# p3achyjr/p3achygo

Measured on AMD Instinct MI355X. Metric: self-play positions/sec at 1/8 MI355X, b12c256btl3 19x19 n=32, higher is better.
Workload: dtype f16; 1 GPU; b12c256btl3 random-init, self-play: C++ host (Gumbel MCTS n=32, default k<=5, selected k=5) -> p3hip_run over batches of 1024 leaf positions -> results back to the search; one step = one round = one engine batch of each of the 8 game groups = 8192 positions; batch_per_gpu=1024, concurrent_games_per_gpu=8192, game_groups_per_gpu=8, lanes_per_group=1, ladder_node_budget=0, parallelism=games sharded x1, no collective

## Files before the change

p3achygo_amd/csrc/engine.cpp:

```cpp
#include <hip/hip_runtime.h>
#include <chrono>

#include <atomic>
#include <cmath>
#include <cstdio>
#include <cstdlib>
#include <cstring>
#include <functional>
#include <map>
#include <memory>
#include <unordered_set>
#include <string>
#include <vector>

#include "../../include/p3hip.h"
#include "kernels.h"
#include "lconv_i8.h"
#include "slot_state.h"
#include "symmetry.h"
#include "transformer.h"

namespace {

constexpr float kBnEps = 1e-3f;
constexpr int kNLoc = 361;
constexpr size_t kFeatBytes = sizeof(p3hip_features);
static_assert(sizeof(p3hip_features) == 1860, "p3hip_features layout");
static_assert(sizeof(p3hip_result) == 4 * 1892, "p3hip_result layout");

thread_local std::string g_create_error;

struct Tensor {
  std::vector<int> dims;
  const float* data;
  size_t size() const {
    size_t n = 1;
    for (int d : dims) n *= d;
    return n;
  }
};

struct WeightFile {
  int version = 0, nblocks = 0, C = 0, Cb = 0, H = 0, V = 0, bint = 0, inner = 0, btype = 0;
  int model_C = 0;
  std::vector<std::vector<float>> padded;
  std::vector<float> data;
  std::map<std::string, Tensor> tensors;

  bool load(const char* path, std::string& err) {
    FILE* f = fopen(path, "rb");
    if (!f) { err = std::string("cannot open ") + path; return false; }
    char magic[4];
    int hdr[10];
    if (fread(magic, 1, 4, f) != 4 || memcmp(magic, "P3W1", 4) != 0 || fread(hdr, 4, 10, f) != 10) {
      err = "not a .p3w file"; fclose(f); return false;
    }
    version = hdr[0]; nblocks = hdr[1]; C = hdr[2]; Cb = hdr[3]; H = hdr[4]; V = hdr[5];
    bint = hdr[6]; inner = hdr[7]; btype = hdr[8];
    int nt = hdr[9];
    if (nt < 1 || nt > 8192 || nblocks < 1 || nblocks > 256 || (btype == 3 ? bint != 0 : bint < 1)) {
      err = "implausible .p3w header"; fclose(f); return false;
    }
    struct Ent { char name[48]; int ndim; int dims[4]; long long off; };
    std::vector<Ent> ents(nt);
    long long total = 0;
    for (auto& e : ents) {
      if (fread(e.name, 1, 48, f) != 48 || fread(&e.ndim, 4, 1, f) != 1 ||
          fread(e.dims, 4, 4, f) != 4 || fread(&e.off, 8, 1, f) != 1) {
        err = "truncated tensor table"; fclose(f); return false;
      }
      long long sz = 1;
      bool ok = e.ndim >= 0 && e.ndim <= 4 && e.off >= 0 && e.off < (1ll << 31);
      for (int d = 0; ok && d < e.ndim; ++d) {
        ok = e.dims[d] > 0 && e.dims[d] < (1 << 24);
        sz *= e.dims[d];
        ok = ok && sz < (1ll << 31);
      }
      if (!ok) { err = "corrupt tensor table"; fclose(f); return false; }
      if (e.off + sz > total) total = e.off + sz;
    }
    long pos = ftell(f);
    pos += (64 - pos % 64) % 64;
    fseek(f, pos, SEEK_SET);
    data.resize(total);
    if (fread(data.data(), 4, total, f) != (size_t)total) { err = "truncated data"; fclose(f); return false; }
    fclose(f);
    for (auto& e : ents) {
      Tensor t;
      t.dims.assign(e.dims, e.dims + e.ndim);
      t.data = data.data() + e.off;
      tensors[std::string(e.name, strnlen(e.name, sizeof e.name))] = t;
    }
    model_C = C;
    if (btype == 3 && p3::tfm_supported(C, Cb) && p3::tfm_stream_width(C) != C) pad_transformer_io(p3::tfm_stream_width(C));
    return true;
  }
  void pad_transformer_io(int Cp) {
    auto pad = [&](const std::string& n, size_t rows, bool out_channels) {
      auto it = tensors.find(n);
      const size_t want = out_channels ? rows * C : (size_t)C * 32;
      if (it == tensors.end() || it->second.size() != want) return;
      std::vector<float> w(out_channels ? rows * Cp : (size_t)Cp * 32, 0.0f);
      for (size_t i = 0; i < want; ++i) {
        const size_t r = out_channels ? i / C : 0, c = out_channels ? i % C : i;
        w[out_channels ? r * Cp + c : c] = it->second.data[i];
      }
      padded.push_back(std::move(w));
      Tensor t;
      t.dims = it->second.dims;
      t.dims.back() = out_channels ? Cp : t.dims.back();
      if (!out_channels) t.dims[t.dims.size() - 2] = Cp;
      t.data = padded.back().data();
      it->second = t;
    };
    pad("init_conv.w", 25 * 15, true);
    pad("init_game.w", 8, true);
    pad("init_game.b", 1, true);
    for (const char* n : {"policy.conv_p.w", "policy.conv_g.w", "value.conv.w"}) pad(n, 0, false);
    C = Cp;
  }
  mutable std::string missing;
  mutable std::vector<std::vector<float>> zeros;
  mutable std::map<std::string, Tensor> stand_ins;
  const Tensor& get(const std::string& n, size_t expect = 0) const {
    auto it = tensors.find(n);
    if (it != tensors.end() && (expect == 0 || it->second.size() == expect)) return it->second;
    if (missing.size() < 400) missing += (missing.empty() ? "" : ", ") + n + (it == tensors.end() ? "" : " (wrong size)");
    auto st = stand_ins.find(n);
    if (st != stand_ins.end()) return st->second;
    zeros.emplace_back(expect ? expect : 1, 0.0f);
    Tensor t;
    t.dims = {(int)zeros.back().size()};
    t.data = zeros.back().data();
    return stand_ins[n] = t;
  }
  bool is_broadcast(int i) const { return bint > 0 && i % bint == bint - 1; }
};

struct Arena {
  std::vector<unsigned char> host;
  bool bad_stream = false;
  size_t add(const void* p, size_t bytes) {
    size_t off = (host.size() + 255) & ~size_t(255);
    host.resize(off + bytes);
    memcpy(host.data() + off, p, bytes);
    return off;
  }
};

void pack_segment(std::vector<_Float16>& dst, const float* W, int taps, int ntaps_pad,
                  int cin_total, int cout_total, int cin0, int CB, int cout0, int CP) {
  for (int tap = 0; tap < ntaps_pad; ++tap)
    for (int q = 0; q < CB / 16; ++q)
      for (int h = 0; h < 2; ++h)
        for (int co = 0; co < CP; ++co)
          for (int e = 0; e < 8; ++e) {
            int ci = cin0 + q * 16 + h * 8 + e, c = cout0 + co;
            float v = 0.0f;
            if (tap < taps && ci < cin_total && c < cout_total)
              v = W[((size_t)tap * cin_total + ci) * cout_total + c];
            dst.push_back((_Float16)v);
          }
}

void pack_segment_3x3(std::vector<_Float16>& dst, const float* W, int cin_total, int cout_total, int CB, int CP) {
  for (int ky = 0; ky < 3; ++ky)
    for (int q32 = 0; q32 < CB / 32; ++q32)
      for (int kx = 0; kx < 3; ++kx)
        for (int q = 2 * q32; q < 2 * q32 + 2; ++q)
          for (int h = 0; h < 2; ++h)
            for (int co = 0; co < CP; ++co)
              for (int e = 0; e < 8; ++e) {
                const int ci = q * 16 + h * 8 + e, tap = ky * 3 + kx;
                float v = 0.0f;
                if (ci < cin_total && co < cout_total) v = W[((size_t)tap * cin_total + ci) * cout_total + co];
                dst.push_back((_Float16)v);
              }
}

void pack_granule(std::vector<_Float16>& dst, const float* W, int cin_total, int cout_total, int tap, int k0, int cout0,
                  const float* scale) {
  for (int j = 0; j < 2; ++j)
    for (int c = 0; c < 2; ++c)
      for (int h = 0; h < 2; ++h)
        for (int n = 0; n < 32; ++n)
          for (int el = 0; el < 8; ++el) {
            const int co = cout0 + 32 * c + n;
            float v = W[((size_t)tap * cin_total + k0 + 16 * j + 8 * h + el) * cout_total + co];
            if (scale) v *= scale[co];
            dst.push_back((_Float16)v);
          }
}

struct FoldedBN { size_t scale_off, shift_off; };

void pack_afrag(std::vector<_Float16>& dst, const float* W, int K, int N, int ld, int col0) {
  for (int ct = 0; ct < N / 16; ++ct)
    for (int st = 0; st < K / 32; ++st)
      for (int lane = 0; lane < 64; ++lane)
        for (int el = 0; el < 8; ++el)
          dst.push_back((_Float16)W[(size_t)(32 * st + 8 * (lane >> 4) + el) * ld + col0 + 16 * ct + (lane & 15)]);
}

void spiral_rope_table(int D, double* cos_out, double* sin_out) {
  const int K = 4, per = D / K, nth = D / 4;
  const double kPi = 3.14159265358979323846;
  std::vector<double> theta(D);
  for (int i = 0; i < D; ++i) {
    const int k = i / per, r = (i % per) / 2;
    int t = 2 * (k % (K / 2)) + (r / 2) * K + (r % 2);
    if (t > nth - 1) t = nth - 1;
    theta[i] = std::pow(100.0, -(double)t / nth);
  }
  for (int s = 0; s < kNLoc; ++s)
    for (int i = 0; i < D; ++i) {
      const double ang = (i / per) * (kPi / K);
      const double proj = (s / 19) * std::cos(ang) + (s % 19) * std::sin(ang);
      cos_out[s * D + i] = std::cos(theta[i] * proj);
      sin_out[s * D + i] = std::sin(theta[i] * proj);
    }
}

struct LayerPlan {
  int kw, cin, cout;
  bool pre, act, res, dual;
  FoldedBN pre_bn, out_bn;
  int in_buf, out_buf, out2_buf;
  size_t stream_off = 0;
  int nms = 0;
  size_t q_off = 0, qs_off = 0;
  int qidx = -1;
};

struct TfmPlan { size_t rms_in = 0, rms_out = 0, wqkv = 0, wo = 0, wgu = 0, wdown = 0; };

struct BlockPlan {
  int kind;
  TfmPlan tfm;
  std::vector<LayerPlan> layers;
  size_t stream_off = 0;
  int nms = 0;
  size_t stream_bytes = 0;
  FoldedBN bn[p3::kMaxBlockLayers];
  size_t stream2_off = 0, stream3_off = 0;
  int nms2 = 0, nms3 = 0;
  size_t dense_bias_off = 0;
  bool first_fused = false, last_fused = false;
  bool dense_fused = false;
  int head_of = -1, tail_of = -1;
  size_t head_bytes = 0, tail_bytes = 0;
};

struct Pass {
  const unsigned char* feats = nullptr;
  int npos = 0;
  float* out = nullptr;
  float* res = nullptr;
  int* timed = nullptr;
};

}

struct p3hip_engine {
  std::string path, err;
  int batch = 0, device = 0;
  uint32_t flags = 0;
  WeightFile wf;
  int n_cu = 256;
  bool c128_wg8 = false;
  bool runs_contiguous = false;
  bool bcast_fuse = true;
  int stop_block = -1;
  bool fuse = true, join = true;
  int stagger = -1;
  bool pair_turns = true;
  bool direct_results = true;
  bool time_run = false;
  bool blockw = false;
  bool blockw_diag = false;
  struct BlockwRun { size_t first; int nblk; size_t stream_off, prm_off; };
  std::vector<BlockwRun> bw_runs;
  hipModule_t bw_mod = nullptr;
  hipFunction_t bw_fn = nullptr;
  unsigned long long* d_bw_stamps = nullptr;
  hipStream_t stream = nullptr;
  hipGraph_t graph = nullptr;
  hipGraphExec_t graph_exec = nullptr;
  bool graph_failed = false, graph_warm = false;
  Pass graph_pass;
  std::vector<hipEvent_t> blk_ev;

  unsigned char* d_arena = nullptr;
  std::vector<BlockPlan> blocks;
  size_t init_stream_off = 0; int init_nms = 0;
  size_t game_w_off = 0, game_b_off = 0;
  size_t heads_stream_off = 0; int heads_nms = 0;
  size_t heads_conv_a_off = 0, heads_image_off = 0;
  bool tfm = false;
  int tfm_heads = 0, tfm_D = 0;
  size_t rope_cos_off = 0, rope_sin_off = 0;
  bool int8 = false, calibrating = false, have_scales = false;
  int n_q = 0;
  unsigned* d_amax = nullptr;
  float* d_ascale = nullptr;
  std::vector<float> h_scale;
  bool sym = false;
  uint32_t sym_mask = 0xFF;
  int sym_k = 8;
  int sym_syms[p3::kNumSyms] = {0, 1, 2, 3, 4, 5, 6, 7};
  int rows = 0;
  unsigned char* d_sfeats = nullptr;
  float* d_cout = nullptr;
  bool heads_fused = false;
  std::map<std::string, size_t> head_off;

  unsigned char* h_feats = nullptr;
  unsigned char* h_feats_compact = nullptr;
  unsigned char* d_feats = nullptr;
  _Float16 *d_x = nullptr, *d_t = nullptr, *d_u = nullptr;
  _Float16* d_qkv = nullptr;
#ifdef P3_DIAG
  unsigned long long* d_stamps = nullptr;
  unsigned long long* d_spans = nullptr;
  int launch_index = 0;
#endif
  _Float16* d_s = nullptr;
  float* d_hp = nullptr;
  float* d_out = nullptr;
  float* h_out = nullptr;
  float* d_res = nullptr;
  double t_h2d = 0, t_fwd = 0, t_d2h = 0;
  long t_runs = 0;
  bool feats_identity = false;
  p3::SlotStates slots;
  int last_n = 0;
  std::vector<unsigned char> slot_sym, row_sym;

  struct DeviceCache {
    bool on = false;
    unsigned mask = 0, run = 0;
    unsigned long long* d_tkeys = nullptr;
    unsigned* d_tmeta = nullptr;
    float* d_tvals = nullptr;
    p3::CacheKey* h_slot_keys = nullptr;
    p3::CacheKey *h_keys = nullptr, *d_keys = nullptr;
    int *h_hit = nullptr, *d_hit = nullptr, *h_victim = nullptr, *d_victim = nullptr;
    int *h_lists = nullptr, *d_lists = nullptr;
    unsigned *h_sym = nullptr, *d_sym = nullptr;
    unsigned char* d_feats2 = nullptr;
    std::vector<int> out_row;
    std::vector<unsigned char> was_hit;
    unsigned long long lookups = 0, hits = 0, inserts = 0;
  } cache;
  int out_row_of(int slot) const {
    const int row = slots.row(slot);
    return (row >= 0 && cache.on) ? cache.out_row[row] : row;
  }

  bool check(hipError_t e, const char* what) {
    if (e == hipSuccess) return true;
    err = std::string(what) + ": " + hipGetErrorString(e);
    return false;
  }
  template <class T>
  const T* dev(size_t off) const { return reinterpret_cast<const T*>(d_arena + off); }
  bool bind() { return check(hipSetDevice(device), "hipSetDevice"); }
};

namespace {

FoldedBN fold_bn(Arena& ar, const WeightFile& wf, const std::string& prefix, size_t n) {
  const Tensor& g = wf.get(prefix + ".gamma", n);
  const Tensor& b = wf.get(prefix + ".beta", n);
  const Tensor& m = wf.get(prefix + ".mean", n);
  const Tensor& v = wf.get(prefix + ".var", n);
  std::vector<float> sc(n), sh(n);
  for (size_t i = 0; i < n; ++i) {
    sc[i] = g.data[i] / std::sqrt(v.data[i] + kBnEps);
    sh[i] = b.data[i] - m.data[i] * sc[i];
  }
  FoldedBN f;
  f.scale_off = ar.add(sc.data(), n * 4);
  f.shift_off = ar.add(sh.data(), n * 4);
  return f;
}

size_t add_stream(Arena& ar, const std::vector<_Float16>& s, int& nms, int cout_pass) {
  const size_t ms = (size_t)cout_pass * 128;
  if (s.size() * 2 % ms != 0) ar.bad_stream = true;
  nms = (int)(s.size() * 2 / ms);
  return ar.add(s.data(), s.size() * 2);
}

bool build_plan(p3hip_engine* e, Arena& ar) {
  const WeightFile& wf = e->wf;
  const int C = wf.C, Cb = wf.Cb;
  const bool fused = (C == 256 && Cb == 128) || (C == 128 && Cb == 64);
  const bool classic = wf.btype == 2 && C == 192 && wf.inner == 2;
  const bool bottleneck_ok = wf.btype == 1 || (wf.btype == 0 && wf.inner >= 1 && wf.inner <= 3);
  const bool layerwise = (C == 384 && Cb == 192 && bottleneck_ok) || classic;
  const bool v_ok = wf.V == 32 || wf.V == 48 || wf.V == 64 || wf.V == 80;
  const bool tfm = wf.btype == 3 && p3::tfm_supported(wf.model_C, Cb) && C == p3::tfm_stream_width(wf.model_C) &&
                   (C == 384 || p3::heads_fusable(C, wf.V));
  if ((!((fused && bottleneck_ok) || layerwise) && !tfm) || wf.H != 32 || !v_ok) {
    e->err = "unsupported architecture for the HIP engine (need (C, Cb) in {(128,64), (256,128), (384,192)} with "
             "btl (1-3 inner layers) or nbt blocks, or C=192 classic blocks of two convs, or a transformer trunk "
             "(" P3HIP_TRANSFORMER_SET "); H=32, V in {32,48,64,80} (transformer: V in {32,48,64}, and 80 at d > 256))";
    return false;
  }
  e->tfm = tfm;
  if (tfm) {
    e->tfm_heads = Cb;
    e->tfm_D = wf.model_C / Cb;
  }
  if (e->int8 && !layerwise) {
    e->err = "INT8 is available only for layer-wise trunks (C = 384 / C_b = 192 btl or nbt blocks, C = 192 classic "
             "blocks); this trunk runs fused block kernels or the transformer";
    return false;
  }
  const int CB = classic ? 64 : ((layerwise || tfm) ? 128 : Cb);
  const int CPI = classic ? 64 : 128;
  {
    std::vector<_Float16> s;
    const Tensor& w = wf.get("init_conv.w", (size_t)25 * 15 * C);
    for (int cp = 0; cp < C / CPI; ++cp)
      pack_segment(s, w.data, 25, 28, 15, C, 0, 16, cp * CPI, CPI);
    e->init_stream_off = add_stream(ar, s, e->init_nms, CPI);
    e->game_w_off = ar.add(wf.get("init_game.w", (size_t)8 * C).data, 8 * C * 4);
    e->game_b_off = ar.add(wf.get("init_game.b", (size_t)C).data, C * 4);
  }
  {
    static const bool want_blockw = getenv("P3HIP_BLOCKW") != nullptr && atoi(getenv("P3HIP_BLOCKW")) != 0;
    e->blockw = want_blockw && C == 256 && Cb == 128 && wf.btype == 0 && wf.inner >= 1 && wf.inner <= 3;
    if (e->blockw) e->bcast_fuse = false;
  }
  bool have_xa = false;
  std::vector<std::pair<size_t, std::vector<_Float16>>> run_streams;
  std::vector<_Float16> head_stream, tail_stream;
  int head_of = -1, tail_of = -1;
  std::vector<std::function<void()>> layout;
  auto flush_run = [&]() {
    if (!run_streams.empty()) {
      auto rs_all = std::make_shared<std::vector<std::pair<size_t, std::vector<_Float16>>>>(std::move(run_streams));
      auto hs = std::make_shared<std::vector<_Float16>>(std::move(head_stream));
      auto ts = std::make_shared<std::vector<_Float16>>(std::move(tail_stream));
      const int h_of = head_of, t_of = tail_of;
      layout.push_back([&ar, e, rs_all, hs, ts, h_of, t_of, Cb]() {
        int nms_unused = 0;
        if (h_of >= 0) {
          add_stream(ar, *hs, nms_unused, Cb);
          BlockPlan& b = e->blocks[rs_all->front().first];
          b.head_of = h_of;
          b.head_bytes = hs->size() * 2;
          e->blocks[h_of].last_fused = true;
        }
        for (auto& rs : *rs_all) {
          BlockPlan& b = e->blocks[rs.first];
          b.stream_off = add_stream(ar, rs.second, b.nms, Cb);
          b.stream_bytes = rs.second.size() * 2;
        }
        if (t_of >= 0) {
          add_stream(ar, *ts, nms_unused, Cb);
          BlockPlan& b = e->blocks[rs_all->back().first];
          b.tail_of = t_of;
          b.tail_bytes = ts->size() * 2;
        }
      });
    }
    run_streams.clear();
    head_stream.clear();
    tail_stream.clear();
    head_of = tail_of = -1;
  };
  if (tfm) {
    std::vector<double> cd(kNLoc * e->tfm_D), sd(kNLoc * e->tfm_D);
    spiral_rope_table(e->tfm_D, cd.data(), sd.data());
    const std::vector<float> cf(cd.begin(), cd.end()), sf(sd.begin(), sd.end());
    e->rope_cos_off = ar.add(cf.data(), cf.size() * 4);
    e->rope_sin_off = ar.add(sf.data(), sf.size() * 4);
  }
  for (int i = 0; tfm && i < wf.nblocks; ++i) {
    const std::string p = "blocks." + std::to_string(i);
    const int c = wf.model_C, f = 2 * c;
    auto T = [&](const char* n, size_t sz) { return wf.get(p + "." + n, sz).data; };
    BlockPlan bp;
    bp.kind = 5;
    bp.tfm.rms_in = ar.add(T("rms_in.scale", c), c * 4);
    bp.tfm.rms_out = ar.add(T("rms_out.scale", c), c * 4);
    std::vector<_Float16> w;
    for (const char* n : {"q.w", "k.w", "v.w"}) pack_afrag(w, T(n, (size_t)c * c), c, c, c, 0);
    bp.tfm.wqkv = ar.add(w.data(), w.size() * 2);
    w.clear();
    pack_afrag(w, T("o.w", (size_t)c * c), c, c, c, 0);
    bp.tfm.wo = ar.add(w.data(), w.size() * 2);
    w.clear();
    pack_afrag(w, T("ffn_gate.w", (size_t)c * f), c, f, f, 0);
    pack_afrag(w, T("ffn_up.w", (size_t)c * f), c, f, f, 0);
    bp.tfm.wgu = ar.add(w.data(), w.size() * 2);
    w.clear();
    pack_afrag(w, T("ffn_down.w", (size_t)f * c), f, c, c, 0);
    bp.tfm.wdown = ar.add(w.data(), w.size() * 2);
    e->blocks.push_back(bp);
  }
  for (int i = 0; !tfm && i < wf.nblocks; ++i) {
    BlockPlan bp;
    if (layerwise) flush_run();
    const std::string p = "blocks." + std::to_string(i);
    auto W = [&](int j, int kw, int cin, int cout) {
      return wf.get(p + ".conv" + std::to_string(j) + ".w", (size_t)kw * kw * cin * cout).data;
    };
    if (wf.is_broadcast(i)) {
      bp.kind = 3;
      have_xa = false;
      bp.bn[0] = fold_bn(ar, wf, p + ".bn0", C);
      bp.bn[1] = fold_bn(ar, wf, p + ".bn1", C);
      const int CPb = (CB == 128) ? 128 : 64;
      std::vector<_Float16> s0, s1, s2;
      for (int cp = 0; cp < C / CPb; ++cp)
        for (int ip = 0; ip < C / CB; ++ip) {
          pack_segment(s0, W(0, 1, C, C), 1, 1, C, C, ip * CB, CB, cp * CPb, CPb);
          pack_segment(s2, W(1, 1, C, C), 1, 1, C, C, ip * CB, CB, cp * CPb, CPb);
        }
      const Tensor& dw = wf.get(p + ".dense.w", (size_t)kNLoc * kNLoc);
      for (int jp = 0; jp < 3; ++jp)
        for (int q = 0; q < 24; ++q)
          for (int h = 0; h < 2; ++h)
            for (int jj = 0; jj < 128; ++jj)
              for (int el = 0; el < 8; ++el) {
                int ii = q * 16 + h * 8 + el, j = jp * 128 + jj;
                float v = (ii < kNLoc && j < kNLoc) ? dw.data[(size_t)ii * kNLoc + j] : 0.0f;
                s1.push_back((_Float16)v);
              }
      const bool fused_neighbours = fused && e->bcast_fuse;
      std::vector<_Float16> f0, f2;
      if (fused_neighbours)
        for (int cp = 0; cp < 2; ++cp)
          for (int k = 0; k < 2; ++k) {
            const int ip = cp == 0 ? k : 1 - k;
            pack_segment(f0, W(0, 1, C, C), 1, 1, C, C, ip * Cb, Cb, cp * Cb, Cb);
            pack_segment(f2, W(1, 1, C, C), 1, 1, C, C, ip * Cb, Cb, cp * Cb, Cb);
          }
      if (fused_neighbours && !run_streams.empty()) {
        tail_stream = f0;
        tail_of = i;
        bp.first_fused = true;
        static const bool no_dfuse = getenv("P3HIP_NO_DFUSE") != nullptr;
        if (C == 256 && Cb == 128 && wf.btype == 0 && !no_dfuse) {
          bp.dense_fused = true;
          std::vector<_Float16> dpad;
          for (int jp = 0; jp < 3; ++jp)
            for (int q = 0; q < 24; ++q)
              for (int h = 0; h < 2; ++h)
                for (int jj = 0; jj < 128; ++jj)
                  for (int el = 0; el < 8; ++el) {
                    const int r = q * 16 + h * 8 + el, y = r / 20, x = r % 20, j = jp * 128 + jj;
                    const bool on_board = x < 19 && y < 19;
                    float v = (on_board && j < kNLoc) ? dw.data[(size_t)(y * 19 + x) * kNLoc + j] : 0.0f;
                    dpad.push_back((_Float16)v);
                  }
          tail_stream.clear();
          for (int cp = 0; cp < 2; ++cp) {
            for (int ip = 0; ip < 2; ++ip) pack_segment(tail_stream, W(0, 1, C, C), 1, 1, C, C, ip * Cb, Cb, cp * Cb, Cb);
            tail_stream.insert(tail_stream.end(), dpad.begin(), dpad.end());
          }
        }
      }
      flush_run();
      if (fused_neighbours && i + 1 < wf.nblocks && !wf.is_broadcast(i + 1)) {
        head_stream = f2;
        head_of = i;
      }
      bp.stream_off = add_stream(ar, s0, bp.nms, CPb);
      bp.stream2_off = add_stream(ar, s1, bp.nms2, 128);
      bp.stream3_off = add_stream(ar, s2, bp.nms3, CPb);
      bp.dense_bias_off = ar.add(wf.get(p + ".dense.b", (size_t)kNLoc).data, kNLoc * 4);
    } else if (layerwise) {
      bp.kind = 4;
      const int nconv = classic ? 2 : ((wf.btype == 0) ? wf.inner + 2 : 6);
      for (int j = 0; j < nconv; ++j) bp.bn[j] = fold_bn(ar, wf, p + ".bn" + std::to_string(j), (classic || j == 0) ? C : Cb);
      FoldedBN next_bn0{};
// ... 221 lines not shown
    a.tail_scale[0] = e->dev<float>(bb.bn[0].scale_off);
    a.tail_shift[0] = e->dev<float>(bb.bn[0].shift_off);
    if (bb.dense_fused) {
      a.tail_dense = 1;
      a.uout = a.uout2 = e->d_u;
      a.dense_bias[0] = e->dev<float>(bb.dense_bias_off);
      a.dense_scale[0] = e->dev<float>(bb.bn[1].scale_off);
      a.dense_shift[0] = e->dev<float>(bb.bn[1].shift_off);
    }
    a.nms_total += (int)(lb.tail_bytes / ms_bytes);
  }
  {
    const bool long_launch = npos >= 3 * e->n_cu * (e->wf.C == 256 || e->c128_wg8 ? 1 : 2);
    const bool shared = (e->flags & P3HIP_FLAG_SHARED_DEVICE) != 0;
    a.stagger = e->stagger >= 0 ? e->stagger : ((a.head || a.tail) && long_launch && !shared ? 10000 : 0);
    a.pair_turns = e->pair_turns && e->wf.C == 128 && !e->c128_wg8 && npos >= 4 * e->n_cu;
  }
  for (int b = 0; b < count; ++b) {
    const BlockPlan& bp = e->blocks[first + b];
    a.nms_total += (int)(bp.stream_bytes / ms_bytes);
    for (int j = 0; j < p3::kMaxBlockLayers; ++j) {
      a.blk[b].scale[j] = e->dev<float>(bp.bn[j].scale_off);
      a.blk[b].shift[j] = e->dev<float>(bp.bn[j].shift_off);
    }
  }
  return a;
}

int joined_launch(p3hip_engine* e, size_t first, int npos, p3::BlockArgs* out) {
  if (!e->join || !e->runs_contiguous) return 0;
  std::vector<std::pair<size_t, int>> runs;
  size_t bi = first;
  int nb = 0;
  while (bi < e->blocks.size() && (int)runs.size() < p3::kMaxRuns) {
    const int kind = e->blocks[bi].kind;
    if (kind != 0) break;
    int n = 1;
    while (bi + n < e->blocks.size() && e->blocks[bi + n].kind == kind) ++n;
    if (n > p3::kMaxFuse || nb + n > p3::kMaxLaunchBlocks) break;
    runs.emplace_back(bi, n);
    nb += n;
    bi += n;
    if (bi + 1 < e->blocks.size() && e->blocks[bi].kind == 3 && e->blocks[bi].first_fused && e->blocks[bi].last_fused &&
        e->blocks[bi].dense_fused && e->blocks[bi + 1].kind == 0) ++bi;
    else break;
  }
  if (runs.size() < 2) return 0;
  const size_t last_run_end = runs.back().first + runs.back().second;
  p3::BlockArgs a = block_args(e, runs[0].first, runs[0].second, npos);
  a.nruns = (int)runs.size();
  a.nms_total = 0;
  a.tail = 0;
  a.tail_dense = 1;
  const bool closed = !a.head && !(e->blocks[runs.back().first + runs.back().second - 1].tail_of >= 0);
  _Float16* other = closed ? e->d_t : e->d_u;
  a.zin2 = e->d_u;
  a.uout = other;
  a.zin = other;
  a.uout2 = e->d_u;
  const size_t ms_bytes = (size_t)p3::block_macro_step_bytes(e->wf.C, e->c128_wg8);
  int k = 0;
  for (size_t r = 0; r < runs.size(); ++r) {
    a.run_nblk[r] = runs[r].second;
    const BlockPlan& fb = e->blocks[runs[r].first];
    const BlockPlan& lb = e->blocks[runs[r].first + runs[r].second - 1];
    if (fb.head_of >= 0) a.nms_total += (int)(fb.head_bytes / ms_bytes);
    for (int b = 0; b < runs[r].second; ++b, ++k) {
      const BlockPlan& bp = e->blocks[runs[r].first + b];
      a.nms_total += (int)(bp.stream_bytes / ms_bytes);
      for (int j = 0; j < p3::kMaxBlockLayers; ++j) {
        a.blk[k].scale[j] = e->dev<float>(bp.bn[j].scale_off);
        a.blk[k].shift[j] = e->dev<float>(bp.bn[j].shift_off);
      }
    }
    if (r + 1 < runs.size() || lb.tail_of >= 0) {
      const BlockPlan& bb = e->blocks[lb.tail_of];
      a.nms_total += (int)(lb.tail_bytes / ms_bytes);
      a.tail_scale[r] = e->dev<float>(bb.bn[0].scale_off);
      a.tail_shift[r] = e->dev<float>(bb.bn[0].shift_off);
      a.dense_bias[r] = e->dev<float>(bb.dense_bias_off);
      a.dense_scale[r] = e->dev<float>(bb.bn[1].scale_off);
      a.dense_shift[r] = e->dev<float>(bb.bn[1].shift_off);
      if (r + 1 == runs.size()) a.tail = 1;
    }
  }
  for (size_t r = 0; r + 1 < runs.size(); ++r) {
    const BlockPlan& lb = e->blocks[runs[r].first + runs[r].second - 1];
    const BlockPlan& nf = e->blocks[runs[r + 1].first];
    if (lb.stream_off + lb.stream_bytes + lb.tail_bytes + nf.head_bytes != nf.stream_off) return 0;
  }
  *out = a;
  return (int)(last_run_end - first);
}

int fused_run(const p3hip_engine* e, size_t first) {
  const int kind = e->blocks[first].kind;
  if (kind != 0 && kind != 1) return 0;
  int n = 1;
  while (e->fuse && n < p3::kMaxFuse && first + n < e->blocks.size() && e->blocks[first + n].kind == kind) ++n;
  return n;
}

extern "C" const unsigned char p3_blockw_hsaco[];
extern "C" const unsigned char p3_blockw_hsaco_end[];
struct BlockwArgs {
  const void* x; const void* ws; const void* prm;
  int npos, nblk, nwg, pad;
  void* stamps;
  unsigned long long pad2[2];
};
static_assert(sizeof(BlockwArgs) == 64, "kernarg layout of k_blockw");

bool load_blockw(p3hip_engine* e) {
  if (e->bw_fn) return true;
  if (!e->check(hipModuleLoadData(&e->bw_mod, p3_blockw_hsaco), "hipModuleLoadData k_blockw")) return false;
  const std::string name = "k_blockw_L" + std::to_string(e->wf.inner) + (e->blockw_diag ? "_diag" : "");
  if (!e->check(hipModuleGetFunction(&e->bw_fn, e->bw_mod, name.c_str()), "hipModuleGetFunction k_blockw")) return false;
  if (e->blockw_diag) {
    constexpr size_t bytes = 8 * 16 * 4 * 24 * 8;
    if (!e->check(hipMalloc((void**)&e->d_bw_stamps, bytes), "hipMalloc stamps") ||
        !e->check(hipMemsetAsync(e->d_bw_stamps, 0, bytes, e->stream), "hipMemset stamps")) return false;
  }
  return true;
}

bool launch_blockw(p3hip_engine* e, const p3hip_engine::BlockwRun& run, int npos) {
  if (!load_blockw(e)) return false;
  BlockwArgs a{};
  a.x = e->d_x;
  a.ws = e->d_arena + run.stream_off;
  a.prm = e->d_arena + run.prm_off;
  a.npos = npos;
  a.nblk = run.nblk;
  a.nwg = npos < e->n_cu ? npos : e->n_cu;
  a.stamps = e->d_bw_stamps;
  size_t size = sizeof a;
  void* cfg[] = {HIP_LAUNCH_PARAM_BUFFER_POINTER, &a, HIP_LAUNCH_PARAM_BUFFER_SIZE, &size, HIP_LAUNCH_PARAM_END};
  return e->check(hipModuleLaunchKernel(e->bw_fn, a.nwg, 1, 1, 256, 1, 1, 0, e->stream, nullptr, cfg), "launch k_blockw");
}

template <class Launch>
bool timed_launch(p3hip_engine* e, int* timed, Launch&& launch) {
  const bool on = timed && 2 * *timed + 1 < (int)e->blk_ev.size();
  if (on) hipEventRecord(e->blk_ev[2 * *timed], e->stream);
  if (!launch()) return false;
  if (on) hipEventRecord(e->blk_ev[2 * (*timed)++ + 1], e->stream);
  return true;
}

bool enqueue_forward(p3hip_engine* e, const Pass& p) {
  const WeightFile& wf = e->wf;
  const int C = wf.C, npos = p.npos;
  hipStream_t s = e->stream;
  {
    p3::InitArgs a{};
    a.feats = p.feats; a.x = e->d_x; a.npos = npos;
    a.wstream = e->d_arena + e->init_stream_off; a.nms_total = e->init_nms;
    a.game_w = e->dev<float>(e->game_w_off); a.game_b = e->dev<float>(e->game_b_off);
    if (!e->check(p3::launch_init(C, a, grid_for(e, npos, 1), s), "launch k_init")) return false;
  }
#ifdef P3_DIAG
  e->launch_index = 0;
#endif
  const int stop_block = e->stop_block;
  for (size_t bi = 0; bi < e->blocks.size(); ++bi) {
    if (stop_block >= 0 && (int)bi >= stop_block) return true;
    const BlockPlan& bp = e->blocks[bi];
    if (bp.kind == 5) {
      const int d = wf.model_C;
      const size_t per = (size_t)e->rows * p3::kTfmLPad * d;
      _Float16 *q = e->d_qkv, *k = q + per, *v = k + per, *o = e->d_t;
      p3::TfmQkvArgs a{e->d_x, q, k, v, npos, e->dev<float>(bp.tfm.rms_in), e->d_arena + bp.tfm.wqkv,
                       e->dev<float>(e->rope_cos_off), e->dev<float>(e->rope_sin_off)};
      if (!e->check(p3::launch_tfm_qkv(d, e->tfm_D, a, s), "launch k_tfm_qkv")) return false;
      const p3::TfmAttnArgs b{q, k, v, o, npos, e->tfm_heads};
      if (!timed_launch(e, p.timed, [&] { return e->check(p3::launch_tfm_attn(e->tfm_D, b, s), "launch k_tfm_attn"); }))
        return false;
      const p3::TfmFfnArgs f{o, e->d_x, npos, e->d_arena + bp.tfm.wo, e->dev<float>(bp.tfm.rms_out),
                             e->d_arena + bp.tfm.wgu, e->d_arena + bp.tfm.wdown};
      if (!e->check(p3::launch_tfm_ffn(d, f, s), "launch k_tfm_ffn")) return false;
    } else if (bp.kind == 3) {
      p3::Conv1x1Args c0{};
      c0.in = e->d_x; c0.out16 = e->d_t; c0.npos = npos;
      c0.wstream = e->d_arena + bp.stream_off; c0.nms_total = bp.nms;
      c0.scale = e->dev<float>(bp.bn[0].scale_off); c0.shift = e->dev<float>(bp.bn[0].shift_off);
      if (!bp.first_fused && !e->check(p3::launch_conv1x1(C, 0, c0, e->n_cu, s), "launch conv_first")) return false;
      p3::BDenseArgs d{};
      d.t = e->d_t; d.u = e->d_u; d.npos = npos;
      d.wstream = e->d_arena + bp.stream2_off; d.nms_total = bp.nms2;
      d.bias = e->dev<float>(bp.dense_bias_off);
      d.scale = e->dev<float>(bp.bn[1].scale_off); d.shift = e->dev<float>(bp.bn[1].shift_off);
      if (!(bp.first_fused && bp.dense_fused) &&
          !e->check(p3::launch_bdense(C, d, grid_for(e, npos, 1), s), "launch bdense")) return false;
      p3::Conv1x1Args c1{};
      c1.in = e->d_u; c1.out16 = e->d_x; c1.npos = npos;
      c1.wstream = e->d_arena + bp.stream3_off; c1.nms_total = bp.nms3;
      if (!bp.last_fused && !e->check(p3::launch_conv1x1(C, 1, c1, e->n_cu, s), "launch conv_last")) return false;
    } else if (bp.kind == 4) {
      const size_t half = (size_t)e->rows * wf.Cb * kNLoc;
      _Float16* bufs[5] = {e->d_x, e->d_t, e->d_t + half, e->d_u, e->d_u + half};
      auto fill = [&](auto& a, const LayerPlan& lp) {
        a.in = bufs[lp.in_buf]; a.out = bufs[lp.out_buf]; a.npos = npos;
        a.out2 = lp.out2_buf >= 0 ? reinterpret_cast<decltype(a.out2)>(bufs[lp.out2_buf]) : nullptr;
        a.pre = lp.pre; a.act = lp.act; a.res = lp.res; a.dual = lp.dual;
        if (a.pre) { a.scale_in = e->dev<float>(lp.pre_bn.scale_off); a.shift_in = e->dev<float>(lp.pre_bn.shift_off); }
        if (a.act || a.dual) { a.scale_out = e->dev<float>(lp.out_bn.scale_off); a.shift_out = e->dev<float>(lp.out_bn.shift_off); }
      };
      if (e->int8 && !e->calibrating) {
        for (const LayerPlan& lp : bp.layers) {
          p3::LConvI8Args a{};
          fill(a, lp);
          a.w = e->dev<int8_t>(lp.q_off); a.w_scale = e->dev<float>(lp.qs_off);
          a.act_scale = e->d_ascale; a.in_scale = lp.qidx; a.out_scale = lp.qidx + 1;
          auto launch = [&] { return e->check(p3::launch_lconv_i8(lp.kw, lp.cin, lp.cout, a, s), "launch k_lconv_i8"); };
          if (!timed_launch(e, lp.kw == 3 ? p.timed : nullptr, launch)) return false;
        }
        continue;
      }
      for (const LayerPlan& lp : bp.layers) {
        if (e->calibrating) {
          p3::AbsmaxArgs m{};
          m.in = bufs[lp.in_buf]; m.npos = npos; m.C = lp.cin; m.amax = e->d_amax + lp.qidx;
          if (lp.pre) { m.scale = e->dev<float>(lp.pre_bn.scale_off); m.shift = e->dev<float>(lp.pre_bn.shift_off); }
          if (!e->check(p3::launch_absmax(m, e->n_cu, s), "launch k_absmax")) return false;
        }
        p3::LConvArgs a{};
        fill(a, lp);
        a.wstream = e->d_arena + lp.stream_off; a.nms_total = lp.nms;
        auto launch = [&] { return e->check(p3::launch_lconv(lp.kw, lp.cin, lp.cout, a, e->n_cu, s), "launch k_lconv"); };
        if (!timed_launch(e, lp.kw == 3 ? p.timed : nullptr, launch)) return false;
      }
    } else if (e->blockw && bp.kind == 0) {
      const p3hip_engine::BlockwRun* run = nullptr;
      for (const auto& r : e->bw_runs) if (r.first == bi) run = &r;
      if (!run) { e->err = "internal error: no k_blockw run starts at this block"; return false; }
      if (!timed_launch(e, p.timed, [&] { return launch_blockw(e, *run, npos); })) return false;
      bi += run->nblk - 1;
    } else {
      int run = fused_run(e, bi);
      p3::BlockArgs a;
      const int joined = joined_launch(e, bi, npos, &a);
      if (joined > 0) run = joined;
      else a = block_args(e, bi, run, npos);
#ifdef P3_DIAG
      {
        static const int which = getenv("P3DIAG_LAUNCH") ? atoi(getenv("P3DIAG_LAUNCH")) : 1;
        constexpr size_t bytes = (size_t)p3::kStampWgs * 8 * p3::kStampSections * p3::kStampSlots * 8;
        if (!e->d_stamps && hipMalloc((void**)&e->d_stamps, bytes) == hipSuccess) hipMemset(e->d_stamps, 0, bytes);
        constexpr size_t span_bytes = (size_t)p3::kSpanWgs * p3::kSpanSlots * 8;
        if (!e->d_spans && hipMalloc((void**)&e->d_spans, span_bytes) == hipSuccess) hipMemset(e->d_spans, 0, span_bytes);
        static const int which_run = getenv("P3DIAG_RUN") ? atoi(getenv("P3DIAG_RUN")) : 1;
        const int idx = (a.nruns > 1) ? 0 : which;
        a.stamp_run = (a.nruns > 1) ? which_run : 0;
        a.spans = (e->launch_index == idx) ? e->d_spans : nullptr;
        a.stamps = (e->launch_index++ == idx) ? e->d_stamps : nullptr;
      }
#endif
      auto launch = [&] { return e->check(p3::launch_block(C, bp.kind, wf.inner, e->c128_wg8, a, e->n_cu, s), "launch k_block"); };
      if (!timed_launch(e, p.timed, launch)) return false;
      bi += run - 1;
    }
  }
  {
    p3::Conv1x1Args c{};
    c.in = e->d_x; c.out32 = e->d_hp; c.npos = npos;
    c.wstream = e->d_arena + e->heads_stream_off; c.nms_total = e->heads_nms;
    if (!e->heads_fused && !e->check(p3::launch_conv1x1(C, 2, c, e->n_cu, s), "launch head convs")) return false;
    p3::HeadsArgs h{};
    h.x = e->d_x;
    h.conv_a = e->d_arena + e->heads_conv_a_off;
    h.image = e->dev<float>(e->heads_image_off);
    h.hp = e->d_hp; h.out = p.out; h.npos = npos; h.V = wf.V;
    h.res = p.res;
    auto F = [&](const char* n) { return e->dev<float>(e->head_off.at(n)); };
    h.gbn_scale = F("gbn_scale"); h.gbn_shift = F("gbn_shift");
    h.gd_w = F("policy.gpool_dense.w"); h.gd_b = F("policy.gpool_dense.b");
    h.moves_w = F("policy.out_moves.w");
    h.pass_w = F("policy.out_pass.w"); h.pass_b = F("policy.out_pass.b");
    h.opt_moves_w = F("policy.opt_moves.w");
    h.opt_pass_w = F("policy.opt_pass.w"); h.opt_pass_b = F("policy.opt_pass.b");
    h.oq_embed_w = F("value.oq_embed.w"); h.oq_embed_b = F("value.oq_embed.b");
    h.oq_out_w = F("value.oq_out.w"); h.oq_out_b = F("value.oq_out.b");
    h.own_w = F("value.own.w");
    h.gamma_pre_w = F("value.gamma_pre.w"); h.gamma_pre_b = F("value.gamma_pre.b");
    h.gamma_out_w = F("value.gamma_out.w"); h.gamma_out_b = F("value.gamma_out.b");
    h.score_pre_w = F("value.score_pre.w"); h.score_pre_b = F("value.score_pre.b");
    h.score_out_w = F("value.score_out.w"); h.score_out_b = F("value.score_out.b");
    if (e->heads_fused) {
      if (!e->check(p3::launch_headsx(C, h, e->n_cu, s), "launch k_headsx")) return false;
    } else if (!e->check(p3::launch_heads(h, npos, s), "launch k_heads")) return false;
  }
  return true;
}

bool expand_sym(p3hip_engine* e, const unsigned char* src, int n) {
  p3::SymExpandArgs x{};
  x.in = src; x.out = e->d_feats; x.n = n; x.k = e->sym_k;
  for (int j = 0; j < p3::kNumSyms; ++j) x.syms[j] = e->sym_syms[j];
  return e->check(p3::launch_sym_expand(x, e->stream), "launch k_sym_expand");
}

bool enqueue_sym(p3hip_engine* e, const Pass& p) {
  if (!expand_sym(e, p.feats, p.npos) || !enqueue_forward(e, Pass{e->d_feats, p.npos * e->sym_k, e->d_cout})) return false;
  p3::SymReduceArgs r{};
  r.rows = e->d_cout; r.out = p.out; r.res = p.res; r.n = p.npos; r.k = e->sym_k;
  for (int j = 0; j < p3::kNumSyms; ++j) r.syms[j] = e->sym_syms[j];
  return e->check(p3::launch_sym_reduce(r, e->stream), "launch k_sym_reduce");
// ... 628 lines not shown
```

Measured before the change: 219,500 positions/s.

## Add dedicated MFMA stem kernel with register-resident weights and LDS padded board

Replaces the generic streamed init conv (5x5, 15->C) with a specialised persistent kernel for C=128/256. Weights are prepacked into MFMA fragments held in registers, each position's features are expanded into a zero-padded LDS image, and a double buffer overlaps fetching the next position's features with the current MFMA work. The game-feature bias is fused in. This removes weight streaming and padding overhead for the small-K stem, at the cost of a new kernel with hand-written feature decoding that must match the original init kernel exactly.

```diff
diff --git a/p3achygo_amd/csrc/engine.cpp b/p3achygo_amd/csrc/engine.cpp
--- a/p3achygo_amd/csrc/engine.cpp
+++ b/p3achygo_amd/csrc/engine.cpp
@@ -17,6 +17,7 @@
 #include "kernels.h"
 #include "lconv_i8.h"
 #include "slot_state.h"
+#include "stem.h"
 #include "symmetry.h"
 #include "transformer.h"
 
@@ -161,6 +162,17 @@
               v = W[((size_t)tap * cin_total + ci) * cout_total + c];
             dst.push_back((_Float16)v);
           }
+}
+
+void pack_stem(std::vector<_Float16>& dst, const float* W, int C) {
+  for (int ct = 0; ct < C / 16; ++ct)
+    for (int st = 0; st < p3::kStemSteps; ++st)
+      for (int l = 0; l < 64; ++l)
+        for (int e = 0; e < 8; ++e) {
+          const int k = 32 * st + 8 * (l >> 4) + e, tap = k >> 4, ci = k & 15;
+          const float v = (tap < 25 && ci < 15) ? W[((size_t)tap * 15 + ci) * C + 16 * ct + (l & 15)] : 0.0f;
+          dst.push_back((_Float16)v);
+        }
 }
 
 void pack_segment_3x3(std::vector<_Float16>& dst, const float* W, int cin_total, int cout_total, int CB, int CP) {
@@ -293,6 +305,7 @@
   unsigned char* d_arena = nullptr;
   std::vector<BlockPlan> blocks;
   size_t init_stream_off = 0; int init_nms = 0;
+  bool stem = false; size_t stem_off = 0;
   size_t game_w_off = 0, game_b_off = 0;
   size_t heads_stream_off = 0; int heads_nms = 0;
   size_t heads_conv_a_off = 0, heads_image_off = 0;
@@ -423,9 +436,15 @@
   {
     std::vector<_Float16> s;
     const Tensor& w = wf.get("init_conv.w", (size_t)25 * 15 * C);
-    for (int cp = 0; cp < C / CPI; ++cp)
-      pack_segment(s, w.data, 25, 28, 15, C, 0, 16, cp * CPI, CPI);
-    e->init_stream_off = add_stream(ar, s, e->init_nms, CPI);
+    e->stem = p3::stem_supported(C);
+    if (e->stem) {
+      pack_stem(s, w.data, C);
+      e->stem_off = ar.add(s.data(), s.size() * sizeof(_Float16));
+    } else {
+      for (int cp = 0; cp < C / CPI; ++cp)
+        pack_segment(s, w.data, 25, 28, 15, C, 0, 16, cp * CPI, CPI);
+      e->init_stream_off = add_stream(ar, s, e->init_nms, CPI);
+    }
     e->game_w_off = ar.add(wf.get("init_game.w", (size_t)8 * C).data, 8 * C * 4);
     e->game_b_off = ar.add(wf.get("init_game.b", (size_t)C).data, C * 4);
   }
@@ -953,7 +972,13 @@
   const WeightFile& wf = e->wf;
   const int C = wf.C, npos = p.npos;
   hipStream_t s = e->stream;
-  {
+  if (e->stem) {
+    p3::StemArgs a{};
+    a.feats = p.feats; a.x = e->d_x; a.npos = npos;
+    a.wfrag = e->dev<_Float16>(e->stem_off);
+    a.game_w = e->dev<float>(e->game_w_off); a.game_b = e->dev<float>(e->game_b_off);
+    if (!e->check(p3::launch_stem(C, a, e->n_cu, s), "launch k_stem")) return false;
+  } else {
     p3::InitArgs a{};
     a.feats = p.feats; a.x = e->d_x; a.npos = npos;
     a.wstream = e->d_arena + e->init_stream_off; a.nms_total = e->init_nms;
diff --git a/p3achygo_amd/csrc/stem.h b/p3achygo_amd/csrc/stem.h
--- /dev/null
+++ b/p3achygo_amd/csrc/stem.h
@@ -0,0 +1,21 @@
+#pragma once
+#include <hip/hip_runtime.h>
+#include <stdint.h>
+
+namespace p3 {
+
+constexpr int kStemSteps = 13;
+
+struct StemArgs {
+  const void* feats;
+  _Float16* x;
+  int npos;
+  const _Float16* wfrag;
+  const float* game_w;
+  const float* game_b;
+};
+
+bool stem_supported(int C);
+hipError_t launch_stem(int C, const StemArgs& a, int n_cu, hipStream_t s);
+
+}
diff --git a/p3achygo_amd/csrc/stem.hip b/p3achygo_amd/csrc/stem.hip
--- /dev/null
+++ b/p3achygo_amd/csrc/stem.hip
@@ -0,0 +1,175 @@
+#include "stem.h"
+
+#include <stddef.h>
+
+#include "../../include/p3hip.h"
+#include "conv_core.h"
+
+namespace p3 {
+
+namespace {
+
+constexpr int kImgW = kBL + 4;
+constexpr int kImgSlots = kImgW * kImgW;
+constexpr int kImgBytes = kImgSlots * 32;
+constexpr int kTiles = (kNLoc + 15) / 16;
+
+constexpr int kFeatColor = offsetof(p3hip_features, color), kFeatKomi = offsetof(p3hip_features, komi),
+              kFeatBoard = offsetof(p3hip_features, board), kFeatLast = offsetof(p3hip_features, last_moves),
+              kFeatAtari = offsetof(p3hip_features, stones_atari),
+              kFeatTwo = offsetof(p3hip_features, stones_two_liberties),
+              kFeatThree = offsetof(p3hip_features, stones_three_liberties),
+              kFeatLadder = offsetof(p3hip_features, stones_laddered), kFeatSize = sizeof(p3hip_features);
+
+__device__ __forceinline__ constexpr int tap_shift(int t) { return t < 25 ? (t / 5 - 2) * kImgW + (t % 5 - 2) : 0; }
+
+__device__ __forceinline__ int img_slot(int loc) {
+  const int y = (loc * 3450) >> 16;
+  return (y + 2) * kImgW + (loc - y * kBL) + 2;
+}
+
+struct StemFeat {
+  int board, atari, two, three, ladder;
+  int color, last[10];
+  float komi;
+};
+
+__device__ __forceinline__ StemFeat stem_fetch(const void* feats, int pos, int loc) {
+  const unsigned char* f = (const unsigned char*)feats + (size_t)pos * kFeatSize;
+  StemFeat r;
+  r.color = (signed char)f[kFeatColor];
+  r.komi = *(const float*)(f + kFeatKomi);
+#pragma unroll
+  for (int i = 0; i < 10; ++i) r.last[i] = ((const int*)(f + kFeatLast))[i];
+  r.board = r.atari = r.two = r.three = r.ladder = 0;
+  if (loc < kNLoc) {
+    r.board = (signed char)f[kFeatBoard + loc];
+    r.atari = (signed char)f[kFeatAtari + loc];
+    r.two = (signed char)f[kFeatTwo + loc];
+    r.three = (signed char)f[kFeatThree + loc];
+    r.ladder = (signed char)f[kFeatLadder + loc];
+  }
+  return r;
+}
+
+template <int C>
+__device__ __forceinline__ void stem_stage(char* img, float* bias, const StemFeat& f, int loc, const float (&gw)[8],
+                                           float gb) {
+  const int color = f.color;
+  if (loc < kNLoc) {
+    auto our = [&](int v) { return (_Float16)(v == color ? 1.0f : 0.0f); };
+    auto opp = [&](int v) { return (_Float16)(v == -color ? 1.0f : 0.0f); };
+    h8 lo = {our(f.board), opp(f.board), 0, 0, 0, 0, 0, our(f.atari)};
+    const h8 hi = {opp(f.atari), our(f.two), opp(f.two), our(f.three), opp(f.three), our(f.ladder), opp(f.ladder), 0};
+    const int y = (loc * 3450) >> 16, xx = loc - y * kBL;
+#pragma unroll
+    for (int m = 0; m < 5; ++m)
+      if (f.last[2 * m] == y && f.last[2 * m + 1] == xx) lo[2 + m] = (_Float16)1.0f;
+    char* s = img + img_slot(loc) * 32;
+    *(h8*)s = lo;
+    *(h8*)(s + 16) = hi;
+  }
+  if (threadIdx.x < C) {
+    float gsv[8];
+    gsv[0] = color == 1 ? 1.0f : 0.0f;
+    gsv[1] = color == 1 ? 0.0f : 1.0f;
+#pragma unroll
+    for (int m = 0; m < 5; ++m) gsv[2 + m] = (f.last[2 * m] == 19 && f.last[2 * m + 1] == 0) ? 1.0f : 0.0f;
+    gsv[7] = (color == 1 ? -1.0f : 1.0f) * f.komi / 15.0f;
+    float b = gb;
+#pragma unroll
+    for (int k = 0; k < 8; ++k) b += gw[k] * gsv[k];
+    bias[threadIdx.x] = b;
+  }
+}
+
+}
+
+template <int C>
+__global__ void __launch_bounds__(512, 2) k_stem(StemArgs a) {
+  constexpr int NCG = C / 32;
+  constexpr int PS = 8 / NCG;
+  static_assert(NCG * PS == 8, "C = 128 or 256");
+  extern __shared__ __attribute__((aligned(16))) char smem[];
+  float* const bias_lds = (float*)(smem + 2 * kImgBytes);
+  const int tid = threadIdx.x, lane = tid & 63;
+  const int wid = __builtin_amdgcn_readfirstlane(tid >> 6);
+  const int cg = wid % NCG, part = wid / NCG;
+  const int n = lane & 15, q = lane >> 4;
+
+  h8 A[2][kStemSteps];
+#pragma unroll
+  for (int u = 0; u < 2; ++u)
+#pragma unroll
+    for (int s = 0; s < kStemSteps; ++s)
+      A[u][s] = *(const h8*)(a.wfrag + (((size_t)(2 * cg + u) * kStemSteps + s) * 64 + lane) * 8);
+  float gw[8], gb = 0.0f;
+#pragma unroll
+  for (int k = 0; k < 8; ++k) gw[k] = tid < C ? a.game_w[k * C + tid] : 0.0f;
+  if (tid < C) gb = a.game_b[tid];
+  for (int i = tid; i < 2 * kImgBytes / 16; i += 512) ((f32x4*)smem)[i] = f32x4{0.f, 0.f, 0.f, 0.f};
+  __syncthreads();
+
+  int pos = blockIdx.x;
+  stem_stage<C>(smem, bias_lds, stem_fetch(a.feats, pos, tid), tid, gw, gb);
+  for (int buf = 0; pos < a.npos; pos += gridDim.x, buf ^= 1) {
+    __syncthreads();
+    const int next = pos + gridDim.x;
+    StemFeat fn;
+    if (next < a.npos) fn = stem_fetch(a.feats, next, tid);
+    const char* img = smem + buf * kImgBytes + (q & 1) * 16;
+    f32x4 bias[2];
+#pragma unroll
+    for (int u = 0; u < 2; ++u) bias[u] = *(const f32x4*)(bias_lds + buf * C + 32 * cg + 16 * u + 4 * q);
+    _Float16* __restrict__ xo = a.x + (size_t)pos * C * kNLoc + ((size_t)(4 * cg + (q >> 1)) * kNLoc) * 8 + (q & 1) * 4;
+
+    auto bload = [&](h8 (&b)[kStemSteps], int tile) {
+      int loc = tile * 16 + n;
+      if (loc >= kNLoc) loc = kNLoc - 1;
+      const char* src = img + img_slot(loc) * 32;
+#pragma unroll
+      for (int s = 0; s < kStemSteps; ++s)
+        b[s] = *(const h8*)(src + ((q >> 1) ? tap_shift(2 * s + 1) : tap_shift(2 * s)) * 32);
+    };
+#pragma unroll 1
+    for (int tile = part; tile < kTiles; tile += PS) {
+      h8 B[kStemSteps];
+      bload(B, tile);
+      __builtin_amdgcn_sched_barrier(0);
+      f32x4 acc[2] = {{0.f, 0.f, 0.f, 0.f}, {0.f, 0.f, 0.f, 0.f}};
+#pragma unroll
+      for (int s = 0; s < kStemSteps; ++s)
+#pragma unroll
+        for (int u = 0; u < 2; ++u) acc[u] = __builtin_amdgcn_mfma_f32_16x16x32_f16(A[u][s], B[s], acc[u], 0, 0, 0);
+      const int loc = tile * 16 + n;
+      if (loc < kNLoc) {
+#pragma unroll
+        for (int u = 0; u < 2; ++u) {
+          h4 o;
+#pragma unroll
+          for (int i = 0; i < 4; ++i) o[i] = (_Float16)(acc[u][i] + bias[u][i]);
+          *(h4*)(xo + (size_t)u * 2 * kNLoc * 8 + loc * 8) = o;
+        }
+      }
+    }
+    if (next < a.npos) stem_stage<C>(smem + (buf ^ 1) * kImgBytes, bias_lds + (buf ^ 1) * C, fn, tid, gw, gb);
+  }
+}
+
+bool stem_supported(int C) { return C == 128 || C == 256; }
+
+hipError_t launch_stem(int C, const StemArgs& a, int n_cu, hipStream_t s) {
+  const size_t lds = 2 * kImgBytes + 2 * C * sizeof(float);
+  const int grid = a.npos < n_cu ? a.npos : n_cu;
+  if (grid <= 0) return hipSuccess;
+  if (C == 256) {
+    hipLaunchKernelGGL((k_stem<256>), dim3(grid), dim3(512), lds, s, a);
+  } else if (C == 128) {
+    hipLaunchKernelGGL((k_stem<128>), dim3(grid), dim3(512), lds, s, a);
+  } else {
+    return hipErrorInvalidValue;
+  }
+  return hipGetLastError();
+}
+
+}
```

Measured after the change: 215,900 positions/s, median of 2. About the same (-1.6%).
